# libav/libav

Measured on AMD Instinct MI355X. Metric: macroblocks_per_s, higher is better.
Workload: dtype u8

## Files before the change

include/mi355_h264_frame.h:

```cpp
#ifndef MI355_H264_FRAME_H
#define MI355_H264_FRAME_H

#include <stddef.h>
#include <stdint.h>

#ifdef __cplusplus
extern "C" {
#endif

#define MI355_MB_INTRA4x4    0x00000001u
#define MI355_MB_INTRA16x16  0x00000002u
#define MI355_MB_INTRA_PCM   0x00000004u
#define MI355_MB_16x16       0x00000008u
#define MI355_MB_16x8        0x00000010u
#define MI355_MB_8x16        0x00000020u
#define MI355_MB_8x8         0x00000040u
#define MI355_MB_P0L0        0x00001000u
#define MI355_MB_P1L0        0x00002000u
#define MI355_MB_P0L1        0x00004000u
#define MI355_MB_P1L1        0x00008000u
#define MI355_MB_8x8DCT      0x01000000u
#define MI355_MB_INTRA       (MI355_MB_INTRA4x4 | MI355_MB_INTRA16x16 | MI355_MB_INTRA_PCM)

#define MI355_MBF_LEFT_EDGE  0x01
// ... 58 lines not shown
#define MI355_H264_MAX_SLOTS 32

typedef struct mi355_h264_slice {
    uint8_t use_weight;
    uint8_t use_weight_chroma;
    uint8_t luma_log2_weight_denom;
    uint8_t chroma_log2_weight_denom;
    uint8_t list_count;
    uint8_t reserved[3];
    uint8_t ref_slot[2][MI355_H264_MAX_REFS];
    int16_t luma_weight[MI355_H264_MAX_REFS][2][2];
    int16_t chroma_weight[MI355_H264_MAX_REFS][2][2][2];
    int16_t implicit_weight[MI355_H264_MAX_REFS][MI355_H264_MAX_REFS];
    uint8_t chroma_qp_table[2][52];
    int16_t implicit_weight_field[2][2 * MI355_H264_MAX_REFS][2 * MI355_H264_MAX_REFS];
} mi355_h264_slice;

typedef struct mi355_h264_frame {
    int32_t mb_width, mb_height;
    uint8_t *dst[3];
    int32_t dst_stride[2];
    uint8_t *recon[3];
    int32_t recon_stride[2];
    const uint8_t *ref[MI355_H264_MAX_SLOTS][3];
    const mi355_h264_mb *mb;
    const int16_t *mv[2];
    const int16_t *coef;
    const mi355_h264_slice *slices;
    int32_t nslices;
    int32_t max_intra_level;
    const uint32_t *intra_list;
    const int32_t *intra_level_start;
    int32_t max_level_width;
    int32_t field_picture;
    int32_t surface_layout;
    int32_t flags;
} mi355_h264_frame;
#define MI355_FRAME_NO_INTER 1
#define MI355_FRAME_MBAFF    2

#define MI355_SURFACE_LINEAR 0
#define MI355_SURFACE_TILED  1
#define MI355_LAYOUTS_LINEAR 1
#define MI355_LAYOUTS_TILED  2
#define MI355_TILE_LUMA_BYTES   256
#define MI355_TILE_CHROMA_BYTES 128

typedef struct mi355_surface_job {
    uint8_t *lin[3];
    uint8_t *tiled[2];
    int32_t lin_stride[2];
    int32_t tiled_stride[2];
    int32_t mb_width, mb_height;
    int32_t to_tiled;
    int32_t reserved0;
} mi355_surface_job;
int mi355_h264_surface_convert_dev(const mi355_surface_job *jobs, int n, int max_mb_width, int max_mb_height, void *stream);

int mi355_h264_decode_frames(const mi355_h264_frame *frames, int nframes, void *stream);

int mi355_h264_decode_frames_dev(const mi355_h264_frame *d_frames, int nframes,
                                 int max_mb_width, int max_mb_height, int max_intra_level,
                                 int max_level_width, void *stream);

int mi355_h264_decode_frames_levels_dev(const mi355_h264_frame *d_frames, int nframes,
                                        int max_mb_width, int max_mb_height, int max_intra_level,
                                        const int32_t *level_widths, void *stream);

int mi355_h264_decode_frames_layouts_dev(const mi355_h264_frame *d_frames, int nframes,
                                         int max_mb_width, int max_mb_height, int max_intra_level,
                                         const int32_t *level_widths, int layouts, void *stream);

int mi355_h264_decode_frames_wide_dev(const mi355_h264_frame *d_frames, int nframes, int max_mb_width, int max_mb_height,
                                      int max_intra_level, const int32_t *level_widths, int bit_depth, int chroma_format_idc,
                                      int passes, void *stream);

int mi355_h264_recon_intra_levels_dev(const mi355_h264_frame *d_frames, int nframes, int max_intra_level, const int32_t *level_widths, void *stream);
int mi355_h264_recon_intra_all_dev(const mi355_h264_frame *d_frames, int nframes, int max_mb_width, int max_mb_height, int max_intra_level, const int32_t *level_widths, void *stream);
int mi355_h264_recon_intra_plan(int max_mb_width, int max_mb_height, int max_intra_level, const int32_t *level_widths, int pinned, int *single, long long *per_picture);
int mi355_h264_recon_inter_dev(const mi355_h264_frame *d_frames, int nframes, int max_mb_width, int max_mb_height, void *stream);
int mi355_h264_recon_inter_layouts_dev(const mi355_h264_frame *d_frames, int nframes, int max_mb_width, int max_mb_height, int layouts, void *stream);
int mi355_h264_recon_run_plan(int nframes, int max_mb_width, int max_mb_height, int forced, int *run, int *runs_row);
int mi355_h264_recon_inter_run_dev(const mi355_h264_frame *d_frames, int nframes, int max_mb_width, int max_mb_height, int run, void *stream);
int mi355_h264_recon_inter_sparse_dev(const mi355_h264_frame *d_frames, int nframes, int max_mb_width, int max_mb_height, void *stream);
int mi355_h264_recon_intra_dev(const mi355_h264_frame *d_frames, int nframes, int max_intra_level, int max_level_width, void *stream);
int mi355_h264_deblock_dev(const mi355_h264_frame *d_frames, int nframes, int max_mb_width, int max_mb_height, void *stream);
int mi355_h264_deblock_layouts_dev(const mi355_h264_frame *d_frames, int nframes, int max_mb_width, int max_mb_height, int layouts, void *stream);

typedef struct mi355_h264_deblock_plan_info {
    int32_t tiled_waves;
    int32_t linear_bands;
    int32_t skip_tiled;
    int32_t linear_launches;
} mi355_h264_deblock_plan_info;
int mi355_h264_deblock_plan(int nframes, int max_mb_width, int max_mb_height, int layouts, int cus, mi355_h264_deblock_plan_info *plan);
int mi355_h264_deblock_form_dev(const mi355_h264_frame *d_frames, int nframes, int max_mb_width, int max_mb_height, int layouts,
                                int tiled_waves, int linear_bands, void *stream);

int mi355_h264_intra_schedule(mi355_h264_mb *mb, int mb_width, int mb_height,
                              uint32_t *list, int32_t *level_start, int *max_level_width);

int mi355_h264_intra_schedule_mbaff(mi355_h264_mb *mb, int mb_width, int mb_height,
                                    uint32_t *list, int32_t *level_start, int *max_level_width);

void *mi355_malloc(size_t bytes);
void  mi355_free(void *dptr);
int   mi355_memcpy_h2d(void *dst, const void *src, size_t bytes);
int   mi355_memcpy_d2h(void *dst, const void *src, size_t bytes);
int   mi355_memcpy_d2d(void *dst, const void *src, size_t bytes);
int   mi355_sync(void *stream);
void  mi355_prefer_blocking_sync(int on);
void *mi355_host_alloc(size_t bytes);
void  mi355_host_free(void *p);
int   mi355_memcpy_h2d_async(void *dst, const void *src, size_t bytes, void *stream);
int   mi355_memcpy_d2h_async(void *dst, const void *src, size_t bytes, void *stream);
int   mi355_memcpy2d_d2h_async(void *dst, size_t dst_pitch, const void *src, size_t src_pitch, size_t width_bytes, size_t rows, void *stream);
int   mi355_memcpy2d_d2d_async(void *dst, size_t dst_pitch, const void *src, size_t src_pitch, size_t width_bytes, size_t rows, void *stream);
int   mi355_event_sync(void *event);
typedef struct mi355_copy_job {
    const void *src;
    void *dst;
    uint64_t bytes;
} mi355_copy_job;
int   mi355_copy_batch_dev(const mi355_copy_job *jobs, int n, size_t max_bytes, void *stream);
typedef struct mi355_h264_pipelines mi355_h264_pipelines;
mi355_h264_pipelines *mi355_h264_pipelines_create(int shares, int turns);
void mi355_h264_pipelines_destroy(mi355_h264_pipelines *p);
int  mi355_h264_pipelines_decode_dev(mi355_h264_pipelines *p, const mi355_h264_frame *d_frames, int nframes, int max_mb_width, int max_mb_height,
                                     int max_intra_level, const int32_t *level_widths, int layouts);
int  mi355_h264_pipelines_sync(mi355_h264_pipelines *p);
int  mi355_h264_pipelines_share(const mi355_h264_pipelines *p, int nframes, int share, int *first, int *count);
void mi355_h264_pipelines_timing(mi355_h264_pipelines *p, int on);
void mi355_h264_pipelines_join(mi355_h264_pipelines *p, int mode);
int  mi355_h264_pipelines_collect(mi355_h264_pipelines *p, double sums[3], int *launches);

void *mi355_stream_create(void);
void  mi355_stream_destroy(void *stream);
int   mi355_stream_wait_event(void *stream, void *event);
void *mi355_event_create(void);
void  mi355_event_destroy(void *event);
int   mi355_event_record(void *event, void *stream);
int   mi355_event_query(void *event);
float mi355_event_elapsed_ms(void *start, void *end);

#ifdef __cplusplus
}
#endif
#endif
```

libav_amd/csrc/h264_frame.hip:

```cpp
#include <cstdlib>
#include <vector>
#include "h264_recon_dev.h"
#include "../../include/mi355dsp.h"


namespace {

__attribute__((amdgpu_waves_per_eu(MI355_RECON_WAVES, MI355_RECON_WAVES)))
__global__ void __launch_bounds__(64)
k_recon_inter(const mi355_h264_frame *__restrict__ frames, int max_w, int max_h, unsigned long long inv_w, unsigned long long inv_h, int nblocks, int per_xcd)
{
    __shared__ MbLds s;
    recon_inter_wave<false>(s, frames, max_w, max_h, inv_w, inv_h, nblocks, per_xcd);
}
__attribute__((amdgpu_waves_per_eu(MI355_RECON_WAVES, MI355_RECON_WAVES)))
__global__ void __launch_bounds__(64)
k_recon_inter_sparse(const mi355_h264_frame *__restrict__ frames, int max_w, int max_h, unsigned long long inv_w, unsigned long long inv_h, int nblocks, int per_xcd)
{
    __shared__ MbLds s;
    recon_inter_wave<true>(s, frames, max_w, max_h, inv_w, inv_h, nblocks, per_xcd);
}

constexpr int TP = 32;
constexpr int CP = 16;
// ... 133 lines not shown
            MI355_WAVE_SYNC();
        }
    } else {
        for (int i = 0; i < 16; i++) {
            const int x0 = 4 * blk_x4(i), y0 = 4 * blk_y4(i);
            const int tr_ok = (h.topright_samples_available << i) & 0x8000;
            if (lane < 5) s.ps.T[lane] = TILE(x0 + lane - 1, y0 - 1);
            else if (lane < 9) s.ps.T[lane] = tr_ok ? TILE(x0 + lane - 1, y0 - 1) : TILE(x0 + 3, y0 - 1);
            if (lane >= 32 && lane < 37) s.ps.L[lane - 32] = TILE(x0 - 1, y0 + lane - 33);
            MI355_WAVE_SYNC();
            intra_pred_wave(s.ps, 0, h.u.intra4x4_pred_mode[i], 0, 0, &TILE(x0, y0), TP);
            const int q = lane & 3;
            int c[4], r[4], row;
#pragma unroll
            for (int k2 = 0; k2 < 4; k2++) c[k2] = s.mb.coef[i * 16 + q + 4 * k2];
            idct4_quad(c, q, r, row);
            if (lane < 4 && ((h.nnz_mask >> i) & 1)) add_row4<true>(&TILE(x0, y0 + row), r);
            MI355_WAVE_SYNC();
        }
    }
    if (!(t & MI355_MB_INTRA16x16)) residual_chroma<true>(s.mb, &CTILE(0, 0, 0), &CTILE(1, 0, 0), CP);
    intra_store_mb<TILED, AGENT>(&TILE(0, 0), TP, &CTILE(0, 0, 0), &CTILE(1, 0, 0), CP, fr, mb_x, mb_y);
}
#undef TILE

__global__ void __launch_bounds__(64)
k_recon_intra(const mi355_h264_frame *frames, int level, int width)
{
    __shared__ IntraLds s;
    const int f = blockIdx.x / width, k = blockIdx.x - f * width;
    const mi355_h264_frame &frd = frames[f];
    if (level > frd.max_intra_level) return;
    const int first = mi355_global(frd.intra_level_start)[level - 1], count = mi355_global(frd.intra_level_start)[level] - first;
    if (k >= count) return;
    const int mb_xy = (int)mi355_global(frd.intra_list)[first + k];
    if (uniform(frd.surface_layout) == MI355_SURFACE_TILED) recon_intra_mb<true>(s, frd, mb_xy);
    else recon_intra_mb<false>(s, frd, mb_xy);
}

constexpr int INTRA_SINGLE_LEVELS = 16;
constexpr uint32_t INTRA_NAPS_MAX = 1u << 21;
#ifdef MI355_HIP_EMU_H
static inline uint32_t intra_flag_word(const uint8_t *p) { uint32_t v; std::memcpy(&v, reinterpret_cast<const uint8_t *>(reinterpret_cast<uintptr_t>(p) & ~(uintptr_t)3), 4); return v; }
static inline void intra_flag_set(uint8_t *p) { *p = 1; }
#else
__device__ __forceinline__ uint32_t intra_flag_word(const uint8_t *p) { return agent_load_u32(reinterpret_cast<const uint32_t *>(reinterpret_cast<uintptr_t>(p) & ~(uintptr_t)3)); }
__device__ __forceinline__ void intra_flag_set(uint8_t *p) { __hip_atomic_store(p, (uint8_t)1, __ATOMIC_RELAXED, __HIP_MEMORY_SCOPE_AGENT); }
#endif
__global__ void __launch_bounds__(64)
k_recon_intra_all(const mi355_h264_frame *__restrict__ frames, int nframes, int nmb_max, uint8_t *__restrict__ flags, uint32_t *error_word, uint32_t naps_max)
{
    __shared__ IntraLds s;
    const int k = (int)(blockIdx.x / (unsigned)nframes), f = (int)(blockIdx.x - (unsigned)k * (unsigned)nframes);
    const mi355_h264_frame &frd = frames[f];
    const int nlev = uniform(frd.max_intra_level);
    if (nlev <= 0) return;
    if (k >= uniform(mi355_global(frd.intra_level_start)[nlev])) return;
    const int mb_xy = (int)uniform((int)mi355_global(frd.intra_list)[k]);
    const int W = uniform(frd.mb_width), mb_y = mb_xy / W, mb_x = mb_xy - mb_y * W;
    uint8_t *const pic_flags = mi355_global(flags) + (size_t)f * (size_t)nmb_max;
    const int lane = lane_id();
    const int nx = mb_x + (lane == 3 ? 1 : (lane == 2 ? 0 : -1)), ny = mb_y - (lane == 0 ? 0 : 1);
    const bool inside = lane < 4 && nx >= 0 && nx < W && ny >= 0;
    const int nxy = inside ? ny * W + nx : mb_xy;
    const bool dep = inside && (mi355_global_v(reinterpret_cast<const uint32_t *>(mi355_global(frd.mb) + nxy))[0] & MI355_MB_INTRA) != 0;
    static_assert(offsetof(mi355_h264_mb, mb_type) == 0, "the type word of a record");
    const bool waits = __any(dep);
    if (waits) {
        const uint8_t *fp = pic_flags + nxy;
        const int sh = 8 * (int)(reinterpret_cast<uintptr_t>(fp) & 3);
        uint32_t naps = 0;
        while (__any(dep && ((intra_flag_word(fp) >> sh) & 0xFFu) == 0) && naps < naps_max) { wave_nap(); naps++; }
        if (naps >= naps_max && __any(dep && ((intra_flag_word(fp) >> sh) & 0xFFu) == 0) && lane_id() == 0) atomicOr(error_word, (uint32_t)MI355_ERR_WAIT_EXPIRED);
        MI355_ISSUE_FENCE();
    }
    if (uniform(frd.surface_layout) == MI355_SURFACE_TILED) recon_intra_mb<true, true>(s, frd, mb_xy, waits);
    else recon_intra_mb<false, true>(s, frd, mb_xy, waits);
    agent_drain_stores();
    if (lane == 0 && naps_max) intra_flag_set(pic_flags + mb_xy);
}

}

static int recon_inter_launch(const mi355_h264_frame *d_frames, int nframes, int max_mb_width, int max_mb_height, bool sparse, void *stream, int layouts = MI355_LAYOUTS_LINEAR | MI355_LAYOUTS_TILED, int tiled_run = 0)
{
    if (!mi355::bind() || !d_frames || nframes <= 0) return -1;
    const int per_frame = max_mb_width * max_mb_height;
    if (per_frame <= 0 || per_frame >= (1 << 24)) return -3;
    const int frames_per_launch = ((1 << 24) - 1) / per_frame;
    const unsigned long long one = 1ull << 40;
    for (int f0 = 0; f0 < nframes; f0 += frames_per_launch) {
        const int nf = nframes - f0 < frames_per_launch ? nframes - f0 : frames_per_launch;
        const int nblocks = nf * per_frame, per_xcd = (nblocks + 7) / 8;
        const unsigned long long iw = (one + max_mb_width - 1) / max_mb_width, ih = (one + max_mb_height - 1) / max_mb_height;
        if (sparse)
            hipLaunchKernelGGL(k_recon_inter_sparse, dim3((unsigned)(8 * per_xcd)), dim3(64), 0, (hipStream_t)stream,
                               d_frames + f0, max_mb_width, max_mb_height, iw, ih, nblocks, per_xcd);
        else if (layouts == MI355_LAYOUTS_TILED) {
            if (!mi355::recon_inter_tiled_launch(d_frames + f0, nf, max_mb_width, max_mb_height, (hipStream_t)stream, tiled_run)) return -4;
        }
        else
            hipLaunchKernelGGL(k_recon_inter, dim3((unsigned)(8 * per_xcd)), dim3(64), 0, (hipStream_t)stream,
                               d_frames + f0, max_mb_width, max_mb_height, iw, ih, nblocks, per_xcd);
    }
    return hipGetLastError() == hipSuccess ? 0 : -2;
}
extern "C" int mi355_h264_recon_inter_dev(const mi355_h264_frame *d_frames, int nframes, int max_mb_width, int max_mb_height, void *stream)
{
    return recon_inter_launch(d_frames, nframes, max_mb_width, max_mb_height, false, stream);
}
extern "C" int mi355_h264_recon_inter_layouts_dev(const mi355_h264_frame *d_frames, int nframes, int max_mb_width, int max_mb_height, int layouts, void *stream)
{
    if (!(layouts & (MI355_LAYOUTS_LINEAR | MI355_LAYOUTS_TILED))) return -1;
    return recon_inter_launch(d_frames, nframes, max_mb_width, max_mb_height, false, stream, layouts);
}
extern "C" int mi355_h264_recon_inter_run_dev(const mi355_h264_frame *d_frames, int nframes, int max_mb_width, int max_mb_height, int run, void *stream)
{
    int r, runs_row;
    if (run <= 0 || !mi355::recon_run_plan(nframes, max_mb_width, max_mb_height, run, &r, &runs_row)) return -1;
    return recon_inter_launch(d_frames, nframes, max_mb_width, max_mb_height, false, stream, MI355_LAYOUTS_TILED, run);
}
extern "C" int mi355_h264_recon_inter_sparse_dev(const mi355_h264_frame *d_frames, int nframes, int max_mb_width, int max_mb_height, void *stream)
{
    return recon_inter_launch(d_frames, nframes, max_mb_width, max_mb_height, true, stream);
}

extern "C" int mi355_h264_recon_intra_dev(const mi355_h264_frame *d_frames, int nframes, int max_intra_level, int max_level_width, void *stream)
{
    if (!mi355::bind() || !d_frames || nframes <= 0) return -1;
    if (max_intra_level <= 0 || max_level_width <= 0) return 0;
    for (int level = 1; level <= max_intra_level; level++)
        hipLaunchKernelGGL(k_recon_intra, dim3((unsigned)(nframes * max_level_width)), dim3(64), 0, (hipStream_t)stream,
                           d_frames, level, max_level_width);
    return hipGetLastError() == hipSuccess ? 0 : -2;
}

static bool recon_intra_plan(int max_mb_width, int max_mb_height, int max_intra_level, const int32_t *level_widths, int pinned, long long *per_picture)
{
    *per_picture = 0;
    if (pinned == 0 || (pinned != 1 && max_intra_level < INTRA_SINGLE_LEVELS)) return false;
    long long sum = 0;
    for (int level = 1; level <= max_intra_level; level++) sum += level_widths[level - 1] > 0 ? level_widths[level - 1] : 0;
    const long long nmb = (long long)max_mb_width * max_mb_height;
    *per_picture = sum > nmb ? nmb : sum;
    return true;
}
static int intra_single_pin()
{
    static const int single = std::getenv("MI355_INTRA_SINGLE") ? std::atoi(std::getenv("MI355_INTRA_SINGLE")) : -1;
    return single;
}
extern "C" int mi355_h264_recon_intra_plan(int max_mb_width, int max_mb_height, int max_intra_level, const int32_t *level_widths, int pinned, int *single, long long *per_picture)
{
    if (max_mb_width <= 0 || max_mb_height <= 0 || max_intra_level < 0 || (max_intra_level > 0 && !level_widths) || !single || !per_picture) return -1;
    *single = recon_intra_plan(max_mb_width, max_mb_height, max_intra_level, level_widths, pinned < 0 ? intra_single_pin() : pinned, per_picture) ? 1 : 0;
    return 0;
}

extern "C" int mi355_h264_recon_intra_all_dev(const mi355_h264_frame *d_frames, int nframes, int max_mb_width, int max_mb_height, int max_intra_level, const int32_t *level_widths, void *stream)
{
    if (!mi355::bind() || !d_frames || nframes <= 0 || max_mb_width <= 0 || max_mb_height <= 0 || (max_intra_level > 0 && !level_widths)) return -1;
    long long per_picture = 0;
    if (!recon_intra_plan(max_mb_width, max_mb_height, max_intra_level, level_widths, intra_single_pin(), &per_picture))
        return mi355_h264_recon_intra_levels_dev(d_frames, nframes, max_intra_level, level_widths, stream);
    if (per_picture <= 0) return 0;
    const long long nmb = (long long)max_mb_width * max_mb_height;
    if ((long long)nframes * per_picture > 0x7FFFFFFFLL || (long long)nframes * nmb > 0x7FFFFFFFLL) return -3;
    const size_t bytes = ((size_t)nframes * (size_t)nmb + 3) & ~(size_t)3;
    uint32_t *flags = mi355::sync_words((hipStream_t)stream, bytes / 4);
    if (!flags) return -4;
    MI355_TRY(hipMemsetAsync(flags, 0, bytes, (hipStream_t)stream), -4);
    uint32_t *err = mi355::error_word();
    if (!err) return -4;
    static const uint32_t naps_max = std::getenv("MI355_INTRA_NAPS_MAX") ? (uint32_t)std::strtoul(std::getenv("MI355_INTRA_NAPS_MAX"), nullptr, 0) : INTRA_NAPS_MAX;
    hipLaunchKernelGGL(k_recon_intra_all, dim3((unsigned)(nframes * per_picture)), dim3(64), 0, (hipStream_t)stream, d_frames, nframes, (int)nmb, reinterpret_cast<uint8_t *>(flags), err, naps_max);
    return hipGetLastError() == hipSuccess ? 0 : -2;
}

extern "C" int mi355_h264_recon_intra_levels_dev(const mi355_h264_frame *d_frames, int nframes, int max_intra_level, const int32_t *level_widths, void *stream)
{
    if (!mi355::bind() || !d_frames || nframes <= 0 || (max_intra_level > 0 && !level_widths)) return -1;
    for (int level = 1; level <= max_intra_level; level++) {
        const int width = level_widths[level - 1];
        if (width <= 0) continue;
        if ((long long)nframes * width > 0x7FFFFFFFLL) return -3;
        hipLaunchKernelGGL(k_recon_intra, dim3((unsigned)(nframes * width)), dim3(64), 0, (hipStream_t)stream, d_frames, level, width);
    }
    return hipGetLastError() == hipSuccess ? 0 : -2;
}

#ifdef MI355_PROF
extern "C" void mi355_debug_rprof(unsigned long long *out, int reset)
{
    unsigned long long z[16] = {};
    MI355_CHECK(hipDeviceSynchronize());
    MI355_CHECK(hipMemcpyFromSymbol(out, HIP_SYMBOL(g_rprof), sizeof(z)));
    if (reset) MI355_CHECK(hipMemcpyToSymbol(HIP_SYMBOL(g_rprof), z, sizeof(z)));
}
#endif

extern "C" int mi355_h264_decode_frames_dev(const mi355_h264_frame *d_frames, int nframes, int max_mb_width, int max_mb_height,
                                            int max_intra_level, int max_level_width, void *stream)
{
// ... 279 lines not shown
```

libav_amd/csrc/h264_frame_dev.h:

```cpp
#ifndef MI355_H264_FRAME_DEV_H
#define MI355_H264_FRAME_DEV_H

#include "mi355_rt.h"
#include "h264_dev.h"
#include "../../include/mi355_h264_frame.h"

namespace mi355 {

typedef uint32_t mi355_u32x4 __attribute__((vector_size(16)));
typedef uint32_t mi355_u32x2 __attribute__((vector_size(8)));
typedef uint32_t mi355_u32x4u __attribute__((vector_size(16), aligned(4)));
typedef uint32_t mi355_u32x2u __attribute__((vector_size(8), aligned(4)));

__device__ __forceinline__ int blk_x4(int i) { return (i & 1) + 2 * ((i >> 2) & 1); }
__device__ __forceinline__ int blk_y4(int i) { return ((i >> 1) & 1) + 2 * (i >> 3); }
__device__ __forceinline__ int blk_index(int x4, int y4) { return (x4 & 1) + 2 * (y4 & 1) + 4 * (x4 >> 1) + 8 * (y4 >> 1); }

__device__ __forceinline__ uint32_t tile_y_off(int mb_x, int mb_y, int stride) { return (uint32_t)(__mul24(mb_y, stride) + mb_x * MI355_TILE_LUMA_BYTES); }
__device__ __forceinline__ uint32_t tile_c_off(int mb_x, int mb_y, int stride) { return (uint32_t)(__mul24(mb_y, stride) + mb_x * MI355_TILE_CHROMA_BYTES); }

__device__ __forceinline__ uint4 lds16(const uint8_t *p)
{
    const uint2 a = reinterpret_cast<const uint2 *>(p)[0], b = reinterpret_cast<const uint2 *>(p)[1];
    return make_uint4(a.x, a.y, b.x, b.y);
}
__device__ __forceinline__ void lds16(uint8_t *p, uint4 v)
{
    reinterpret_cast<mi355_u32x2 *>(p)[0] = mi355_u32x2{ v.x, v.y };
    reinterpret_cast<mi355_u32x2 *>(p)[1] = mi355_u32x2{ v.z, v.w };
}
__device__ __forceinline__ uint4 ld16(const uint8_t *p, bool al)
{
    if (al) return *reinterpret_cast<const uint4 *>(p);
    const uint32_t *w = reinterpret_cast<const uint32_t *>(p);
    return make_uint4(w[0], w[1], w[2], w[3]);
}
__device__ __forceinline__ void st16(uint8_t *p, uint4 v, bool al)
{
    if (al) { *reinterpret_cast<mi355_u32x4 *>(p) = mi355_u32x4{ v.x, v.y, v.z, v.w }; return; }
    uint32_t *w = reinterpret_cast<uint32_t *>(p);
    w[0] = v.x; w[1] = v.y; w[2] = v.z; w[3] = v.w;
}
__device__ __forceinline__ uint2 ld8(const uint8_t *p, bool al)
{
    if (al) return *reinterpret_cast<const uint2 *>(p);
    const uint32_t *w = reinterpret_cast<const uint32_t *>(p);
    return make_uint2(w[0], w[1]);
}
__device__ __forceinline__ void st8(uint8_t *p, uint2 v, bool al)
{
    if (al) { *reinterpret_cast<mi355_u32x2 *>(p) = mi355_u32x2{ v.x, v.y }; return; }
    uint32_t *w = reinterpret_cast<uint32_t *>(p);
    w[0] = v.x; w[1] = v.y;
}

bool recon_run_plan(int nframes, int max_w, int max_h, int forced, int *run, int *runs_row);
bool recon_inter_tiled_launch(const mi355_h264_frame *d_frames, int nframes, int max_w, int max_h, hipStream_t stream, int forced_run = 0);
void recon_inter_rest_launch(const mi355_h264_frame *d_frames, int max_w, int max_h, int run, int runs_row, unsigned long long inv_runs, unsigned long long inv_h, int nruns,
                             const uint32_t *rest, hipStream_t stream);
uint32_t *sync_words(hipStream_t stream, size_t words);
}
namespace {
#ifdef MI355_HIP_EMU_H
static inline uint32_t agent_load_u32(const uint32_t *p) { return *p; }
static inline void agent_store_u32(uint32_t *p, uint32_t v) { *p = v; }
static inline void agent_store8(uint8_t *p, uint2 v, bool al8) { mi355::st8(p, v, al8); }
static inline void agent_drain_stores() {}
static inline void wave_nap() { std::fprintf(stderr, "k_deblock_tiled: a band waits for a band that has not run (emulator: workgroups run in order)\n"); std::abort(); }
#else
__device__ __forceinline__ uint32_t agent_load_u32(const uint32_t *p) { return __hip_atomic_load(p, __ATOMIC_RELAXED, __HIP_MEMORY_SCOPE_AGENT); }
__device__ __forceinline__ void agent_store_u32(uint32_t *p, uint32_t v) { __hip_atomic_store(p, v, __ATOMIC_RELAXED, __HIP_MEMORY_SCOPE_AGENT); }
__device__ __forceinline__ void agent_store8(uint8_t *p, uint2 v, bool al8)
{
    if (al8) { __hip_atomic_store(reinterpret_cast<unsigned long long *>(p), (unsigned long long)v.x | ((unsigned long long)v.y << 32), __ATOMIC_RELAXED, __HIP_MEMORY_SCOPE_AGENT); return; }
    uint32_t *w = reinterpret_cast<uint32_t *>(p);
    agent_store_u32(w, v.x); agent_store_u32(w + 1, v.y);
}
__device__ __forceinline__ void agent_drain_stores() { asm volatile("s_waitcnt vmcnt(0)" ::: "memory"); }
__device__ __forceinline__ void wave_nap() { __builtin_amdgcn_s_sleep(16); }
#endif
}
#ifdef MI355_HIP_EMU_H
template <bool AGENT> static inline void lds_dma16(const uint8_t *src, uint8_t *lds_base) { std::memcpy(lds_base + 16 * (threadIdx.x & 63), src, 16); }
#else
template <bool AGENT> __device__ __forceinline__ void lds_dma16(const uint8_t *src, uint8_t *lds_base)
{
    typedef __attribute__((address_space(1))) const void *gptr;
    typedef __attribute__((address_space(3))) void *lptr;
    __builtin_amdgcn_global_load_lds((gptr)src, (lptr)lds_base, 16, 0, AGENT ? 16 : 0);
}
#endif
#ifdef MI355_HIP_EMU_H
static inline void lds_dma_wait() {}
#else
__device__ __forceinline__ void lds_dma_wait() { asm volatile("s_waitcnt vmcnt(0)" ::: "memory"); }
#endif

#endif
```

libav_amd/csrc/h264_frame_tiled.hip:

```cpp
#define MI355_PLAIN_LANE 1
#include "h264_recon_fast.h"

#include <cstdlib>

namespace {
__attribute__((amdgpu_waves_per_eu(MI355_RECON_WAVES, MI355_RECON_WAVES)))
__global__ void __launch_bounds__(64)
k_recon_inter_tiled(const mi355_h264_frame *__restrict__ frames, int max_w, int max_h, int run, int runs_row, unsigned long long inv_runs, unsigned long long inv_h, int nwaves, int per_xcd,
                    uint32_t *__restrict__ rest)
{
    __shared__ MbLds s;
    recon_inter_run(s, frames, max_w, max_h, run, runs_row, inv_runs, inv_h, nwaves, per_xcd, rest);
}
}

namespace mi355 {
bool recon_run_plan(int nframes, int max_w, int max_h, int forced, int *run_out, int *runs_row_out)
{
    if (nframes <= 0 || max_w <= 0 || max_h <= 0 || forced < 0) return false;
    const long long mbs = (long long)nframes * max_w * max_h;
    int run = (int)(mbs / (40ll * 8192));
    run = forced > 0 ? forced : (run < 4 ? 4 : (run > 15 ? 15 : run));
    if (run > max_w) run = max_w;
    const int runs_row = (max_w + run - 1) / run;
    run = (max_w + runs_row - 1) / runs_row;
    if (run > 16) return false;
    *run_out = run;
    *runs_row_out = runs_row;
    return true;
}

bool recon_inter_tiled_launch(const mi355_h264_frame *d_frames, int nframes, int max_w, int max_h, hipStream_t stream, int forced_run)
{
    static const int env = std::getenv("MI355_RECON_RUN") ? std::atoi(std::getenv("MI355_RECON_RUN")) : 0;
    static const int forced = env > 0 ? (env < 4 ? 4 : (env > 15 ? 15 : env)) : 0;
    int run, runs_row;
    if (!recon_run_plan(nframes, max_w, max_h, forced_run > 0 ? forced_run : forced, &run, &runs_row)) return false;
    const unsigned long long one = 1ull << 40;
    const long long total = (long long)nframes * max_h * runs_row;
    const int nwaves = (int)total, per_xcd = (nwaves + 7) / 8;
    uint32_t *rest = sync_words(stream, (size_t)nwaves);
    if (!rest) return false;
    const unsigned long long inv_runs = (one + runs_row - 1) / runs_row, inv_h = (one + max_h - 1) / max_h;
    hipLaunchKernelGGL(k_recon_inter_tiled, dim3((unsigned)(8 * per_xcd)), dim3(64), 0, stream, d_frames, max_w, max_h, run, runs_row, inv_runs, inv_h, nwaves, per_xcd, rest);
    recon_inter_rest_launch(d_frames, max_w, max_h, run, runs_row, inv_runs, inv_h, nwaves, rest, stream);
    return true;
}
}

extern "C" int mi355_h264_recon_run_plan(int nframes, int max_mb_width, int max_mb_height, int forced, int *run, int *runs_row)
{
    if (!run || !runs_row) return -1;
    return mi355::recon_run_plan(nframes, max_mb_width, max_mb_height, forced, run, runs_row) ? 0 : -1;
}
```

libav_amd/csrc/h264_recon_fast.h:

```cpp
#ifndef MI355_H264_RECON_FAST_H
#define MI355_H264_RECON_FAST_H

#include "h264_recon_dev.h"

namespace {

#if defined(FQ_MARKS) && !defined(MI355_HIP_EMU_H)
#define FQ_MARK(name) asm volatile("; MARK " name)
#else
#define FQ_MARK(name)
#endif

constexpr int FQ_COEF = (int)offsetof(MbCore, coef);
constexpr int FQ_RS = FQ_COEF + 768;
constexpr int FQ_RSC = FQ_RS + 512;
constexpr int FQ_ST = FQ_RS;
constexpr int FQ_WY = FQ_RS + 768;
constexpr int FQ_WC = FQ_WY + 1024;
constexpr int FQ_PL = FQ_WC + 256;
constexpr int FQ_PLANE = 16 * 24 + 8;
constexpr int FQ_DUMP = FQ_PL + 16 * 24;
constexpr int FQ_WSTEP = FQ_PL + 2 * FQ_PLANE - FQ_WY;
static_assert(FQ_RS == MB_PY_OFF && (FQ_WY % 16) == 0 && (FQ_PL % 8) == 0 && (FQ_WSTEP % 16) == 0 && FQ_WC + FQ_WSTEP + 256 <= (int)sizeof(MbLds), "fast-path regions inside MbLds");
static_assert(FQ_WY + FQ_WSTEP + 48 * 20 + 24 + 16 + 12 <= (int)sizeof(MbLds), "the second half of a transposing product reads window rows 16..20");
// ... 421 lines not shown
    uint8_t *const base = reinterpret_cast<uint8_t *>(&s);
    FQ_MARK("luma_resid");
    if (has_resid) {
        const mi355_u32x2 r = *reinterpret_cast<const mi355_u32x2 *>(base + k.rsy);
        const uint32_t s01 = pk_sat_u8(pk_add(byte_perm(0u, v, 0x0C010C00u), r[0])), s23 = pk_sat_u8(pk_add(byte_perm(0u, v, 0x0C030C02u), r[1]));
        v = byte_perm(s23, s01, 0x05040100u);
    }
    MI355_WAVE_SYNC();
    *reinterpret_cast<uint32_t *>(base + FQ_ST + k.sy) = v;
}
__device__ __forceinline__ void fq_luma(MbLds &s, const FqLane &k, int so2, int pos, bool has_resid) { fq_luma_out(s, k, fq_luma_pred(s, k, so2, pos), has_resid); }

__device__ __forceinline__ uint32_t fq_chroma_pred(MbLds &s, const FqLane &k, int oc, uint32_t wts)
{
    uint8_t *const base = reinterpret_cast<uint8_t *>(&s);
    const uint32_t at = k.c1 + (uint32_t)oc, sh = at & 3u;
    const uint32_t r0 = fq_bytes4(base + (at & ~3u), sh), r1 = fq_bytes4(base + (at & ~3u) + 12, sh);
    const uint32_t d0 = fq_dot4(byte_perm(r1, r0, 0x05040100u), wts, 32u), d1 = fq_dot4(byte_perm(r1, r0, 0x06050201u), wts, 32u);
    return (d0 >> 6) | ((d1 >> 6) << 8);
}
__device__ __forceinline__ void fq_chroma_out(MbLds &s, const FqLane &k, uint32_t two, bool has_resid)
{
    uint8_t *const base = reinterpret_cast<uint8_t *>(&s);
    if (has_resid) two = pk_sat_u8(pk_add(byte_perm(0u, two, 0x0C010C00u), *reinterpret_cast<const uint32_t *>(base + k.rsc)));
    *reinterpret_cast<uint16_t *>(base + FQ_ST + 256 + k.sc) = (uint16_t)two;
}
__device__ __forceinline__ void fq_chroma(MbLds &s, const FqLane &k, int oc, uint32_t wts, bool has_resid) { fq_chroma_out(s, k, fq_chroma_pred(s, k, oc, wts), has_resid); }
__device__ __forceinline__ void fq_store(MbLds &s, uint8_t *ytile, uint8_t *ctile)
{
    const uint8_t *const base = reinterpret_cast<const uint8_t *>(&s);
    const int lane = lane_id();
    if (lane < 24) {
        const mi355_u32x4 v = *reinterpret_cast<const mi355_u32x4 *>(base + FQ_ST + 16 * lane);
        if (lane < 16) *reinterpret_cast<mi355_u32x4 *>(ytile + (uint32_t)(16 * lane)) = v;
        else *reinterpret_cast<mi355_u32x4 *>(ctile + (uint32_t)(16 * lane - 256)) = v;
    }
}

__device__ __forceinline__ void fq_two(MbLds &s, const FqLane &k, const ResidLane &rl, const FqPic &pic, int mb_xy, int mb_x, int mb_y)
{
    fq_kptr h = fq_konst(pic.mb + mb_xy), mv = fq_konst(pic.mv0 + (size_t)mb_xy * 32);
    const uint32_t type = h[0], nnz = h[1], w2 = h[2], w12 = h[12], w14 = h[14];
    const bool vsplit = (type & MI355_MB_8x16) != 0, has_chroma = (w2 & 0x30u) != 0, resid = (nnz & 0xFFFFu) != 0 || has_chroma;
    const int woff = 0;
    const int n1 = vsplit ? 2 : 8, q1 = vsplit ? 8 : 16;
    const FqGeo g0 = fq_geometry(mv[0], mb_x, mb_y, (int8_t)(w14 & 0xFFu), w12 & 0xFFu, pic.hot.mb_width, pic.hot.mb_height);
    const FqGeo g1 = fq_geometry(mv[n1], mb_x, mb_y, (int8_t)((w14 >> q1) & 0xFFu), (w12 >> q1) & 0xFFu, pic.hot.mb_width, pic.hot.mb_height);
    const int set0 = woff, set1 = woff ^ FQ_WSTEP;
    auto issue = [&](const FqGeo &g, int set) {
        const uint64_t need = fq_need(g.a);
        if (g.a & FQA_INSIDE) fq_windows_issue_inside(s, k, pic.desc, pic.hot, (int)((g.a >> 17) & 31u), (int16_t)(g.d & 0xFFFFu), (int16_t)(g.e & 0xFFFFu), (int)g.d >> 16, (int)g.e >> 16, set, need);
        else fq_windows_issue(s, k, pic.desc, pic.hot, (int)((g.a >> 17) & 31u), (int16_t)(g.d & 0xFFFFu), (int16_t)(g.e & 0xFFFFu), (int)g.d >> 16, (int)g.e >> 16, set, need);
    };
    issue(g0, set0);
    issue(g1, set1);
    if (resid) fq_coef_dma(s, k, pic.coef, mb_xy);
    fq_wait_vm0();
    MI355_WAVE_SYNC();
    if (resid) fq_idct(s, k, rl, nnz, has_chroma, pic.mb + mb_xy);
    if ((g0.a | g1.a) & (FQA_PATCH_Y | FQA_PATCH_C)) {
        fq_windows_patch(s, k, (g0.a & FQA_PATCH_Y) != 0, (g0.a & FQA_PATCH_C) != 0, (int16_t)(g0.e & 0xFFFFu), (int)g0.e >> 16, set0, pic.hot.mb_width, fq_need(g0.a));
        fq_windows_patch(s, k, (g1.a & FQA_PATCH_Y) != 0, (g1.a & FQA_PATCH_C) != 0, (int16_t)(g1.e & 0xFFFFu), (int)g1.e >> 16, set1, pic.hot.mb_width, fq_need(g1.a));
    }
    MI355_WAVE_SYNC();
    const int lane = lane_id();
    const bool second_y = vsplit ? lane >= 32 : (lane & 8) != 0, second_c = vsplit ? (lane & 2) != 0 : (lane & 16) != 0;
    uint32_t vy = 0, vc = 0;
#pragma nounroll
    for (int p = 0; p < 2; p++) {
        const uint32_t ga = p ? g1.a : g0.a, gw = p ? g1.wts : g0.wts;
        const int set = p ? set1 : set0;
        const uint32_t y = fq_luma_pred(s, k, (int)(ga & 31u) + set, (int)((ga >> 7) & 15u));
        const uint32_t c = fq_chroma_pred(s, k, (int)((ga >> 5) & 3u) + set, gw);
        if (second_y == (p != 0)) vy = y;
        if (second_c == (p != 0)) vc = c;
    }
    fq_luma_out(s, k, vy, resid);
    fq_chroma_out(s, k, vc, resid);
    MI355_WAVE_SYNC();
    fq_store(s, pic.hot.recon[0] + tile_y_off(mb_x, mb_y, pic.hot.recon_stride[0]), pic.hot.recon[1] + tile_c_off(mb_x, mb_y, pic.hot.recon_stride[1]));
    MI355_WAVE_SYNC();
}

__device__ __forceinline__ void recon_inter_run(MbLds &s, const mi355_h264_frame *__restrict__ frames, int max_w, int max_h, int run, int runs_row,
                                                unsigned long long inv_runs, unsigned long long inv_h, int nwaves, int per_xcd, uint32_t *__restrict__ rest)
{
    const int wave = xcd_linear((int)blockIdx.x, per_xcd);
    if (wave >= nwaves) return;
    const int row = div_magic(wave, inv_runs);
    const int mb_x = (wave - row * runs_row) * run;
    const int f = div_magic(row, inv_h), mb_y = row - f * max_h;
    const int n = max_w - mb_x < run ? max_w - mb_x : run;
    ResidLane rl;
    resid_lane_compute(rl);
    const FqLane k = fq_lane();
    auto picture = [&](int pf, FqPic &pic) -> bool {
        const mi355_h264_frame &frd = frames[pf];
        pic.hot = frame_hot(frd);
        pic.mb = pic.hot.mb; pic.mv0 = pic.hot.mv[0]; pic.coef = pic.hot.coef; pic.desc = &frd;
        return uniform(frd.surface_layout) == MI355_SURFACE_TILED && !(uniform(frd.flags) & MI355_FRAME_NO_INTER);
    };
    FqPic pic;
    const bool pic_ok = picture(f, pic);
    const int n_row = pic_ok && mb_x < pic.hot.mb_width && mb_y < pic.hot.mb_height ? (n < pic.hot.mb_width - mb_x ? n : pic.hot.mb_width - mb_x) : 0;
    uint32_t deferred = 0;
    if (n_row > 0) {
        const int mb_xy0 = mb_y * pic.hot.mb_width + mb_x;
        const FqRun run = fq_describe(pic, mb_xy0, mb_x, mb_y, n_row);
        uint32_t ra = run.a, rw = run.wts, rn = run.nnz, rd = run.d, re = run.e;
        MI355_PIN(ra); MI355_PIN(rw); MI355_PIN(rn); MI355_PIN(rd); MI355_PIN(re);
        bool pre_w = false, pre_c = false;
        uint32_t a = fq_lane_word(ra, 0);
        for (int i = 0; i < n_row; i++) {
            const bool has_next = i + 1 < n_row;
            const uint32_t an = has_next ? fq_lane_word(ra, i + 1) : 0u;
            const int woff = (i & 1) * FQ_WSTEP;
            bool next_w = false, next_c = false;
            if (a & FQA_FAST) {
                auto issue = [&](int m, uint32_t am, int set) {
                    const uint32_t d = fq_lane_word(rd, m), e = fq_lane_word(re, m);
                    const uint64_t need = fq_need(am);
                    if (am & FQA_INSIDE) fq_windows_issue_inside(s, k, pic.desc, pic.hot, (int)((am >> 17) & 31u), (int16_t)(d & 0xFFFFu), (int16_t)(e & 0xFFFFu), (int)d >> 16, (int)e >> 16, set, need);
                    else fq_windows_issue(s, k, pic.desc, pic.hot, (int)((am >> 17) & 31u), (int16_t)(d & 0xFFFFu), (int16_t)(e & 0xFFFFu), (int)d >> 16, (int)e >> 16, set, need);
                };
                FQ_MARK("issue");
                if (!pre_w) issue(i, a, woff);
                if ((a & FQA_RESID) && !pre_c) fq_coef_dma(s, k, pic.coef, mb_xy0 + i);
                next_w = (an & FQA_FAST) != 0;
                if (next_w) issue(i + 1, an, woff ^ FQ_WSTEP);
                if (next_w) fq_wait_vm2(); else fq_wait_vm0();
                MI355_WAVE_SYNC();
                FQ_MARK("idct");
                if (a & FQA_RESID) fq_idct(s, k, rl, fq_lane_word(rn, i), (a & FQA_CHROMA) != 0, pic.mb + (mb_xy0 + i));
                MI355_WAVE_SYNC();
                FQ_MARK("coefnext");
                next_c = next_w && (an & FQA_RESID);
                if (next_c) fq_coef_dma(s, k, pic.coef, mb_xy0 + i + 1);
                if (a & (FQA_PATCH_Y | FQA_PATCH_C)) {
                    const uint32_t e = fq_lane_word(re, i);
                    fq_windows_patch(s, k, (a & FQA_PATCH_Y) != 0, (a & FQA_PATCH_C) != 0, (int16_t)(e & 0xFFFFu), (int)e >> 16, woff, pic.hot.mb_width, fq_need(a));
                    MI355_WAVE_SYNC();
                }
                FQ_MARK("luma");
                fq_luma(s, k, (int)(a & 31u) + woff, (int)((a >> 7) & 15u), (a & FQA_RESID) != 0);
                FQ_MARK("chroma");
                fq_chroma(s, k, (int)((a >> 5) & 3u) + woff, fq_lane_word(rw, i), (a & FQA_RESID) != 0);
                MI355_WAVE_SYNC();
                FQ_MARK("store");
                fq_store(s, pic.hot.recon[0] + tile_y_off(mb_x + i, mb_y, pic.hot.recon_stride[0]), pic.hot.recon[1] + tile_c_off(mb_x + i, mb_y, pic.hot.recon_stride[1]));
                MI355_WAVE_SYNC();
            } else if (!(a & FQA_INTRA)) {
                deferred |= (a & FQA_TWO) ? 0x10000u << i : 1u << i;
            }
            FQ_MARK("tail");
            pre_w = next_w; pre_c = next_c;
            a = an;
        }
    }
    if (lane_id() == 0) rest[wave] = deferred;
}

constexpr int FQ_REST = 8;
__device__ __forceinline__ void recon_inter_rest(MbLds &s, const mi355_h264_frame *__restrict__ frames, int max_w, int max_h, int run, int runs_row,
                                                 unsigned long long inv_runs, unsigned long long inv_h, int nruns, int ngroups, int per_xcd, const uint32_t *__restrict__ rest)
{
    const int g = xcd_linear((int)blockIdx.x, per_xcd);
    if (g >= ngroups) return;
    const int r = FQ_REST * g + (lane_id() & (FQ_REST - 1));
    const uint32_t mine = r < nruns ? rest[r] : 0u;
    if (!__any(mine != 0)) return;
    auto place = [&](int j, int &f, int &mb_x, int &mb_y) {
        const int w = FQ_REST * g + j;
        const int row = div_magic(w, inv_runs);
        mb_x = (w - row * runs_row) * run;
        f = div_magic(row, inv_h); mb_y = row - f * max_h;
    };
    if (__any((mine >> 16) != 0)) {
        ResidLane rl;
        resid_lane_compute(rl);
        const FqLane k = fq_lane();
        for (int j = 0; j < FQ_REST; j++) {
            uint32_t m = fq_lane_word(mine, j) >> 16;
            if (!m) continue;
            int f, mb_x, mb_y;
            place(j, f, mb_x, mb_y);
            const mi355_h264_frame &frd = frames[f];
            if (uniform(frd.surface_layout) != MI355_SURFACE_TILED) continue;
            FqPic pic;
            pic.hot = frame_hot(frd);
            pic.mb = pic.hot.mb; pic.mv0 = pic.hot.mv[0]; pic.coef = pic.hot.coef; pic.desc = &frd;
            while (m) {
                const int i = __builtin_ctz(m);
                m &= m - 1;
                fq_two(s, k, rl, pic, mb_y * pic.hot.mb_width + mb_x + i, mb_x + i, mb_y);
                fq_wait_vm0();
                MI355_WAVE_SYNC();
            }
        }
    }
    for (int j = 0; j < FQ_REST; j++) {
        uint32_t m = fq_lane_word(mine, j) & 0xFFFFu;
        if (!m) continue;
        int f, mb_x, mb_y;
        place(j, f, mb_x, mb_y);
        if (uniform(frames[f].surface_layout) != MI355_SURFACE_TILED) continue;
        while (m) {
            const int i = __builtin_ctz(m);
            m &= m - 1;
            recon_inter_mb<false, true>(s, frames[f], mb_x + i, mb_y);
            fq_wait_vm0();
            MI355_WAVE_SYNC();
        }
    }
}

}
#endif
```

Measured before the change: 1.421 billion.

## Group multiple macroblock runs per wave in tiled inter reconstruction

```diff
diff --git a/include/mi355_h264_frame.h b/include/mi355_h264_frame.h
--- a/include/mi355_h264_frame.h
+++ b/include/mi355_h264_frame.h
@@ -164,6 +164,8 @@
 int mi355_h264_recon_inter_layouts_dev(const mi355_h264_frame *d_frames, int nframes, int max_mb_width, int max_mb_height, int layouts, void *stream);
 int mi355_h264_recon_run_plan(int nframes, int max_mb_width, int max_mb_height, int forced, int *run, int *runs_row);
 int mi355_h264_recon_inter_run_dev(const mi355_h264_frame *d_frames, int nframes, int max_mb_width, int max_mb_height, int run, void *stream);
+int mi355_h264_recon_group_plan(int nframes, int max_mb_width, int max_mb_height, int forced_run, int forced_runs_per_wave, int *run, int *runs_row, int *runs_per_wave, int *groups_row);
+int mi355_h264_recon_inter_group_dev(const mi355_h264_frame *d_frames, int nframes, int max_mb_width, int max_mb_height, int run, int runs_per_wave, void *stream);
 int mi355_h264_recon_inter_sparse_dev(const mi355_h264_frame *d_frames, int nframes, int max_mb_width, int max_mb_height, void *stream);
 int mi355_h264_recon_intra_dev(const mi355_h264_frame *d_frames, int nframes, int max_intra_level, int max_level_width, void *stream);
 int mi355_h264_deblock_dev(const mi355_h264_frame *d_frames, int nframes, int max_mb_width, int max_mb_height, void *stream);
diff --git a/libav_amd/csrc/h264_frame.hip b/libav_amd/csrc/h264_frame.hip
--- a/libav_amd/csrc/h264_frame.hip
+++ b/libav_amd/csrc/h264_frame.hip
@@ -239,7 +239,7 @@
 
 }
 
-static int recon_inter_launch(const mi355_h264_frame *d_frames, int nframes, int max_mb_width, int max_mb_height, bool sparse, void *stream, int layouts = MI355_LAYOUTS_LINEAR | MI355_LAYOUTS_TILED, int tiled_run = 0)
+static int recon_inter_launch(const mi355_h264_frame *d_frames, int nframes, int max_mb_width, int max_mb_height, bool sparse, void *stream, int layouts = MI355_LAYOUTS_LINEAR | MI355_LAYOUTS_TILED, int tiled_run = 0, int tiled_k = 0)
 {
     if (!mi355::bind() || !d_frames || nframes <= 0) return -1;
     const int per_frame = max_mb_width * max_mb_height;
@@ -254,7 +254,7 @@
             hipLaunchKernelGGL(k_recon_inter_sparse, dim3((unsigned)(8 * per_xcd)), dim3(64), 0, (hipStream_t)stream,
                                d_frames + f0, max_mb_width, max_mb_height, iw, ih, nblocks, per_xcd);
         else if (layouts == MI355_LAYOUTS_TILED) {
-            if (!mi355::recon_inter_tiled_launch(d_frames + f0, nf, max_mb_width, max_mb_height, (hipStream_t)stream, tiled_run)) return -4;
+            if (!mi355::recon_inter_tiled_launch(d_frames + f0, nf, max_mb_width, max_mb_height, (hipStream_t)stream, tiled_run, tiled_k)) return -4;
         }
         else
             hipLaunchKernelGGL(k_recon_inter, dim3((unsigned)(8 * per_xcd)), dim3(64), 0, (hipStream_t)stream,
@@ -276,6 +276,12 @@
     int r, runs_row;
     if (run <= 0 || !mi355::recon_run_plan(nframes, max_mb_width, max_mb_height, run, &r, &runs_row)) return -1;
     return recon_inter_launch(d_frames, nframes, max_mb_width, max_mb_height, false, stream, MI355_LAYOUTS_TILED, run);
+}
+extern "C" int mi355_h264_recon_inter_group_dev(const mi355_h264_frame *d_frames, int nframes, int max_mb_width, int max_mb_height, int run, int runs_per_wave, void *stream)
+{
+    int r, runs_row, k, groups_row;
+    if (run <= 0 || runs_per_wave <= 0 || !mi355::recon_group_plan(nframes, max_mb_width, max_mb_height, run, runs_per_wave, &r, &runs_row, &k, &groups_row)) return -1;
+    return recon_inter_launch(d_frames, nframes, max_mb_width, max_mb_height, false, stream, MI355_LAYOUTS_TILED, run, runs_per_wave);
 }
 extern "C" int mi355_h264_recon_inter_sparse_dev(const mi355_h264_frame *d_frames, int nframes, int max_mb_width, int max_mb_height, void *stream)
 {
diff --git a/libav_amd/csrc/h264_frame_dev.h b/libav_amd/csrc/h264_frame_dev.h
--- a/libav_amd/csrc/h264_frame_dev.h
+++ b/libav_amd/csrc/h264_frame_dev.h
@@ -55,7 +55,8 @@
 }
 
 bool recon_run_plan(int nframes, int max_w, int max_h, int forced, int *run, int *runs_row);
-bool recon_inter_tiled_launch(const mi355_h264_frame *d_frames, int nframes, int max_w, int max_h, hipStream_t stream, int forced_run = 0);
+bool recon_group_plan(int nframes, int max_w, int max_h, int forced_run, int forced_k, int *run, int *runs_row, int *kruns, int *groups_row);
+bool recon_inter_tiled_launch(const mi355_h264_frame *d_frames, int nframes, int max_w, int max_h, hipStream_t stream, int forced_run = 0, int forced_k = 0);
 void recon_inter_rest_launch(const mi355_h264_frame *d_frames, int max_w, int max_h, int run, int runs_row, unsigned long long inv_runs, unsigned long long inv_h, int nruns,
                              const uint32_t *rest, hipStream_t stream);
 uint32_t *sync_words(hipStream_t stream, size_t words);
diff --git a/libav_amd/csrc/h264_frame_tiled.hip b/libav_amd/csrc/h264_frame_tiled.hip
--- a/libav_amd/csrc/h264_frame_tiled.hip
+++ b/libav_amd/csrc/h264_frame_tiled.hip
@@ -6,11 +6,11 @@
 namespace {
 __attribute__((amdgpu_waves_per_eu(MI355_RECON_WAVES, MI355_RECON_WAVES)))
 __global__ void __launch_bounds__(64)
-k_recon_inter_tiled(const mi355_h264_frame *__restrict__ frames, int max_w, int max_h, int run, int runs_row, unsigned long long inv_runs, unsigned long long inv_h, int nwaves, int per_xcd,
-                    uint32_t *__restrict__ rest)
+k_recon_inter_tiled(const mi355_h264_frame *__restrict__ frames, int max_w, int max_h, int run, int runs_row, int kruns, int groups_row, unsigned long long inv_groups,
+                    unsigned long long inv_h, int ngroups, int per_xcd, uint32_t *__restrict__ rest)
 {
     __shared__ MbLds s;
-    recon_inter_run(s, frames, max_w, max_h, run, runs_row, inv_runs, inv_h, nwaves, per_xcd, rest);
+    recon_inter_run(s, frames, max_w, max_h, run, runs_row, kruns, groups_row, inv_groups, inv_h, ngroups, per_xcd, rest);
 }
 }
 
@@ -30,20 +30,40 @@
     return true;
 }
 
-bool recon_inter_tiled_launch(const mi355_h264_frame *d_frames, int nframes, int max_w, int max_h, hipStream_t stream, int forced_run)
+static int recon_group_rule(int run, long long nruns)
+{
+    return run <= 4 && nruns >= 40ll * 8192 ? 2 : 1;
+}
+bool recon_group_plan(int nframes, int max_w, int max_h, int forced_run, int forced_k, int *run_out, int *runs_row_out, int *kruns_out, int *groups_row_out)
+{
+    int run, runs_row;
+    if (forced_k < 0 || !recon_run_plan(nframes, max_w, max_h, forced_run, &run, &runs_row)) return false;
+    int k = forced_k > 0 ? forced_k : recon_group_rule(run, (long long)nframes * max_h * runs_row);
+    if (k > runs_row) k = runs_row;
+    if (k > 64 / run) k = 64 / run;
+    *run_out = run;
+    *runs_row_out = runs_row;
+    *kruns_out = k;
+    *groups_row_out = (runs_row + k - 1) / k;
+    return true;
+}
+
+bool recon_inter_tiled_launch(const mi355_h264_frame *d_frames, int nframes, int max_w, int max_h, hipStream_t stream, int forced_run, int forced_k)
 {
     static const int env = std::getenv("MI355_RECON_RUN") ? std::atoi(std::getenv("MI355_RECON_RUN")) : 0;
     static const int forced = env > 0 ? (env < 4 ? 4 : (env > 15 ? 15 : env)) : 0;
-    int run, runs_row;
-    if (!recon_run_plan(nframes, max_w, max_h, forced_run > 0 ? forced_run : forced, &run, &runs_row)) return false;
+    static const int env_k = std::getenv("MI355_RECON_RUNS_PER_WAVE") ? std::atoi(std::getenv("MI355_RECON_RUNS_PER_WAVE")) : 0;
+    static const int forced_env_k = env_k > 0 ? (env_k > 16 ? 16 : env_k) : 0;
+    int run, runs_row, kruns, groups_row;
+    if (!recon_group_plan(nframes, max_w, max_h, forced_run > 0 ? forced_run : forced, forced_k > 0 ? forced_k : forced_env_k, &run, &runs_row, &kruns, &groups_row)) return false;
     const unsigned long long one = 1ull << 40;
-    const long long total = (long long)nframes * max_h * runs_row;
-    const int nwaves = (int)total, per_xcd = (nwaves + 7) / 8;
-    uint32_t *rest = sync_words(stream, (size_t)nwaves);
+    const int nruns = (int)((long long)nframes * max_h * runs_row);
+    const int ngroups = (int)((long long)nframes * max_h * groups_row), per_xcd = (ngroups + 7) / 8;
+    uint32_t *rest = sync_words(stream, (size_t)nruns);
     if (!rest) return false;
-    const unsigned long long inv_runs = (one + runs_row - 1) / runs_row, inv_h = (one + max_h - 1) / max_h;
-    hipLaunchKernelGGL(k_recon_inter_tiled, dim3((unsigned)(8 * per_xcd)), dim3(64), 0, stream, d_frames, max_w, max_h, run, runs_row, inv_runs, inv_h, nwaves, per_xcd, rest);
-    recon_inter_rest_launch(d_frames, max_w, max_h, run, runs_row, inv_runs, inv_h, nwaves, rest, stream);
+    const unsigned long long inv_runs = (one + runs_row - 1) / runs_row, inv_groups = (one + groups_row - 1) / groups_row, inv_h = (one + max_h - 1) / max_h;
+    hipLaunchKernelGGL(k_recon_inter_tiled, dim3((unsigned)(8 * per_xcd)), dim3(64), 0, stream, d_frames, max_w, max_h, run, runs_row, kruns, groups_row, inv_groups, inv_h, ngroups, per_xcd, rest);
+    recon_inter_rest_launch(d_frames, max_w, max_h, run, runs_row, inv_runs, inv_h, nruns, rest, stream);
     return true;
 }
 }
@@ -53,3 +73,8 @@
     if (!run || !runs_row) return -1;
     return mi355::recon_run_plan(nframes, max_mb_width, max_mb_height, forced, run, runs_row) ? 0 : -1;
 }
+extern "C" int mi355_h264_recon_group_plan(int nframes, int max_mb_width, int max_mb_height, int forced_run, int forced_runs_per_wave, int *run, int *runs_row, int *runs_per_wave, int *groups_row)
+{
+    if (!run || !runs_row || !runs_per_wave || !groups_row) return -1;
+    return mi355::recon_group_plan(nframes, max_mb_width, max_mb_height, forced_run, forced_runs_per_wave, run, runs_row, runs_per_wave, groups_row) ? 0 : -1;
+}
diff --git a/libav_amd/csrc/h264_recon_fast.h b/libav_amd/csrc/h264_recon_fast.h
--- a/libav_amd/csrc/h264_recon_fast.h
+++ b/libav_amd/csrc/h264_recon_fast.h
@@ -527,15 +527,18 @@
     MI355_WAVE_SYNC();
 }
 
-__device__ __forceinline__ void recon_inter_run(MbLds &s, const mi355_h264_frame *__restrict__ frames, int max_w, int max_h, int run, int runs_row,
-                                                unsigned long long inv_runs, unsigned long long inv_h, int nwaves, int per_xcd, uint32_t *__restrict__ rest)
+__device__ __forceinline__ void recon_inter_run(MbLds &s, const mi355_h264_frame *__restrict__ frames, int max_w, int max_h, int run, int runs_row, int kruns, int groups_row,
+                                                unsigned long long inv_groups, unsigned long long inv_h, int ngroups, int per_xcd, uint32_t *__restrict__ rest)
 {
     const int wave = xcd_linear((int)blockIdx.x, per_xcd);
-    if (wave >= nwaves) return;
-    const int row = div_magic(wave, inv_runs);
-    const int mb_x = (wave - row * runs_row) * run;
+    if (wave >= ngroups) return;
+    FQ_MARK("perwave");
+    const int row = div_magic(wave, inv_groups);
+    const int r0 = (wave - row * groups_row) * kruns;
+    const int nr = runs_row - r0 < kruns ? runs_row - r0 : kruns;
+    const int mb_x = r0 * run;
     const int f = div_magic(row, inv_h), mb_y = row - f * max_h;
-    const int n = max_w - mb_x < run ? max_w - mb_x : run;
+    const int n = max_w - mb_x < nr * run ? max_w - mb_x : nr * run;
     ResidLane rl;
     resid_lane_compute(rl);
     const FqLane k = fq_lane();
@@ -548,11 +551,13 @@
     FqPic pic;
     const bool pic_ok = picture(f, pic);
     const int n_row = pic_ok && mb_x < pic.hot.mb_width && mb_y < pic.hot.mb_height ? (n < pic.hot.mb_width - mb_x ? n : pic.hot.mb_width - mb_x) : 0;
-    uint32_t deferred = 0;
+    uint32_t ra = FQA_FAST;
     if (n_row > 0) {
+        FQ_MARK("perrun");
         const int mb_xy0 = mb_y * pic.hot.mb_width + mb_x;
-        const FqRun run = fq_describe(pic, mb_xy0, mb_x, mb_y, n_row);
-        uint32_t ra = run.a, rw = run.wts, rn = run.nnz, rd = run.d, re = run.e;
+        const FqRun run_d = fq_describe(pic, mb_xy0, mb_x, mb_y, n_row);
+        ra = run_d.a;
+        uint32_t rw = run_d.wts, rn = run_d.nnz, rd = run_d.d, re = run_d.e;
         MI355_PIN(ra); MI355_PIN(rw); MI355_PIN(rn); MI355_PIN(rd); MI355_PIN(re);
         bool pre_w = false, pre_c = false;
         uint32_t a = fq_lane_word(ra, 0);
@@ -594,15 +599,21 @@
                 FQ_MARK("store");
                 fq_store(s, pic.hot.recon[0] + tile_y_off(mb_x + i, mb_y, pic.hot.recon_stride[0]), pic.hot.recon[1] + tile_c_off(mb_x + i, mb_y, pic.hot.recon_stride[1]));
                 MI355_WAVE_SYNC();
-            } else if (!(a & FQA_INTRA)) {
-                deferred |= (a & FQA_TWO) ? 0x10000u << i : 1u << i;
             }
             FQ_MARK("tail");
             pre_w = next_w; pre_c = next_c;
             a = an;
         }
     }
-    if (lane_id() == 0) rest[wave] = deferred;
+    FQ_MARK("words");
+    const int j = lane_id();
+    const bool other = j < n_row && !(ra & (FQA_FAST | FQA_INTRA));
+    const unsigned long long def_two = __ballot(other && (ra & FQA_TWO)), def_gen = __ballot(other && !(ra & FQA_TWO));
+    if (j < nr) {
+        const int sh = __mul24(j, run);
+        const uint32_t mask = (1u << run) - 1u;
+        rest[(size_t)row * (size_t)runs_row + (size_t)(r0 + j)] = ((uint32_t)(def_gen >> sh) & mask) | (((uint32_t)(def_two >> sh) & mask) << 16);
+    }
 }
 
 constexpr int FQ_REST = 8;
```

Result: no change. 1.437 billion (median of 2 runs) (+1.1%).
